# PytorchConnectomics/pytorch_connectomics

Measured on AMD Instinct MI355X. Metric: voxels/s (train + sliding-window infer), MedNeXt-S 112^3 bf16, higher is better.
Workload: dtype bf16; 1 GPU; Lucchi++ sliding-window inference (configs[1]): MedNeXt-S k3, 165x1024x768 volume, roi 112^3, overlap 0.5, bump blending, sw_batch_size 8, random-init weights; step = one whole-volume EagerSlidingWindowEngine call (TTA off); value = window-voxels/s; sw_batch_size=8, window_pipeline_streams=3

## Files before the change

pytorch_connectomics_amd/csrc/dwconv_mfma_kernels.hip:

```cpp
#include <type_traits>

#include "dwconv_march.h"
#include "pw_common.h"

namespace pytc {

typedef short s4_t __attribute__((ext_vector_type(4)));
typedef unsigned int u32x4_t __attribute__((ext_vector_type(4)));
typedef unsigned int u32x2a4_t __attribute__((ext_vector_type(2), aligned(4)));
typedef __bf16 bf2_t __attribute__((ext_vector_type(2)));
typedef float f2_t __attribute__((ext_vector_type(2)));

constexpr int MF_TY = 8, MF_TX = 8, MF_CG = 32;
constexpr int MF_EY = MF_TY + 2, MF_EX = MF_TX + 2;
constexpr int MF_EXP = 16;
constexpr int MF_CS = MF_EY * MF_EXP + 2;
constexpr int MF_IMG = MF_CG * MF_CS;
constexpr int MF_NCHUNK = MF_EY * MF_EX * (MF_CG / 8);
constexpr int MF_CPT = 2;
constexpr int MF_TS = 32;
constexpr int MF_RS = MF_TX * MF_TS + 8;

__device__ __forceinline__ unsigned short mf_bf16_bits(float f) {
  unsigned int u = __float_as_uint(f);
  u += 0x7FFFu + ((u >> 16) & 1u);
  return (unsigned short)(u >> 16);
}
__device__ __forceinline__ float mf_bf16_float(unsigned short h) { return __uint_as_float(((unsigned int)h) << 16); }

template <int N>
__device__ __forceinline__ void mf_wait_vm() { asm volatile("s_waitcnt vmcnt(%0)" : : "n"(N) : "memory"); }


template <int N>
__device__ __forceinline__ void mf_wait_vm_upto(int n) {
  if constexpr (N > 0) {
    if (n >= N) { mf_wait_vm<N>(); return; }
    mf_wait_vm_upto<N - 1>(n);
  } else {
    mf_wait_vm<0>();
  }
}

template <int PF, bool LO, int PROBE = 0, bool STORE = true, int MIXHC = 0>
__global__ void __launch_bounds__(256, MIXHC ? 3 : 4)
dwconv3d_k3_mfma_kernel(const unsigned short* __restrict__ x, unsigned short* __restrict__ y, const float* __restrict__ w,
                        const float* __restrict__ bias, float* __restrict__ stats, DwMarch g, DwMix mx) {
  static_assert(PF == 2 || PF == 3, "two or three planes in flight");
  static_assert(MIXHC == 0 || (STORE && PF == 3), "the fused block keeps the output tile and three planes in flight");
  constexpr bool MIX = MIXHC > 0;
  __shared__ __attribute__((aligned(16))) bf16x8_t w2s[MIX ? MIXHC * 2 * 64 : 1];
  __shared__ __attribute__((aligned(16))) h8_t w3s[MIX ? 2 * MIXHC * 64 : 1];
  __shared__ __attribute__((aligned(16))) float mbias[MIX ? 32 * MIXHC + 32 : 4];
  __shared__ __attribute__((aligned(16))) unsigned short image[2][MF_IMG];
  __shared__ __attribute__((aligned(16))) unsigned short otile[STORE ? 2 : 1][STORE ? MF_TY * MF_RS : 8];
  __shared__ float wl[27 * MF_CG];
  __shared__ float red[4][2][16];

  const int tid = threadIdx.x, wave = tid >> 6, lane = tid & 63;
  int b = g.swizzle ? xcd_swizzle(blockIdx.x, gridDim.x) : blockIdx.x;
  const int ncg = g.C / MF_CG;
  const int cg = g.cg_inner ? b % ncg : (b / g.slots) % ncg;
  const int slot_id = g.cg_inner ? (b / ncg) % g.slots : b % g.slots;
  const int n = b / (ncg * g.slots);
  b = slot_id;
  const int fx = b % g.tx; b /= g.tx;
  const int fy = b % g.ty;
  const int zchunk = b / g.ty;
  const int y0 = fy * MF_TY, x0 = fx * MF_TX;
  const int zs = zchunk * g.zc;
  const int ze = min(zs + g.zc, g.D);
  const int C = g.C;
  const long plane_elems = (long)g.H * g.W * C;
  const unsigned short* xn = x + (long)n * g.D * plane_elems + cg * MF_CG;
  unsigned short* yn = y + (long)n * g.D * plane_elems + cg * MF_CG;
  const bool inner = y0 >= 1 && y0 + MF_TY + 1 <= g.H && x0 >= 1 && x0 + MF_TX + 1 <= g.W;

  for (int i = tid; i < 27 * MF_CG; i += 256) wl[i] = w[(long)(i / MF_CG) * C + cg * MF_CG + (i % MF_CG)];
  if constexpr (MIX) {
    const bf16x8_t* w2g = mx.w2n + (long)n * mx.w2_stride;
    for (int i = tid; i < MIXHC * 2 * 64; i += 256) { w2s[i] = w2g[i]; w3s[i] = mx.w3[i]; }
    if (tid < 32 * MIXHC) mbias[tid] = mx.b2n[(long)n * (32 * MIXHC) + tid];
    else if (tid < 32 * MIXHC + 32) mbias[tid] = mx.b3[tid - 32 * MIXHC];
  }
  __syncthreads();

  int goff[MF_CPT], loff[MF_CPT];
  bool cok[MF_CPT];
#pragma unroll
  for (int i = 0; i < MF_CPT; ++i) {
    const int c = tid + 256 * i;
    const int vox = c >> 2, part = c & 3;
    const int yy = vox / MF_EX, xx = vox % MF_EX;
    const int gy = y0 - 1 + yy, gx = x0 - 1 + xx;
    cok[i] = (c < MF_NCHUNK) && gy >= 0 && gy < g.H && gx >= 0 && gx < g.W;
    const int gyc = min(max(gy, 0), g.H - 1), gxc = min(max(gx, 0), g.W - 1);
    goff[i] = (gyc * g.W + gxc) * C + part * 8;
    loff[i] = (c < MF_NCHUNK) ? (part * 8) * MF_CS + yy * MF_EXP + xx : -1;
  }
  u32x4_t stg[PF][MF_CPT];
  auto issue = [&](int gz, u32x4_t (&st)[MF_CPT]) {
    const int zc = min(max(gz, 0), g.D - 1);
#pragma unroll
    for (int i = 0; i < MF_CPT; ++i) {
      const unsigned short* ptr = xn + (long)zc * plane_elems + goff[i];
      asm volatile("global_load_dwordx4 %0, %1, off" : "=&v"(st[i]) : "v"(ptr) : "memory");
    }
  };
  auto landed = [&](u32x4_t (&st)[MF_CPT], int younger) {
    mf_wait_vm_upto<2 * MF_CPT + 2>(younger);
    asm volatile("" : "+v"(st[0]), "+v"(st[1]) : : "memory");
  };
  auto commit = [&](int slot, u32x4_t (&st)[MF_CPT], int gz) {
    const bool zok = gz >= 0 && gz < g.D;
#pragma unroll
    for (int i = 0; i < MF_CPT; ++i) {
      if (loff[i] < 0) continue;
      unsigned short* dst = &image[slot][loff[i]];
      if (inner && zok) {
#pragma unroll
        for (int q = 0; q < 4; ++q) {
          dst[(2 * q) * MF_CS] = (unsigned short)(st[i][q] & 0xffffu);
          dst[(2 * q + 1) * MF_CS] = (unsigned short)(st[i][q] >> 16);
        }
      } else {
        const bool ok = zok && cok[i];
#pragma unroll
        for (int q = 0; q < 4; ++q) {
          const unsigned int dw = ok ? st[i][q] : 0u;
          dst[(2 * q) * MF_CS] = (unsigned short)(dw & 0xffffu);
          dst[(2 * q + 1) * MF_CS] = (unsigned short)(dw >> 16);
        }
      }
    }
  };

  const int h = wave & 1, ph = wave >> 1;
  const int cl = lane >> 2, j = lane & 3;
  const int ch = h * 16 + cl;
  s4_t a_hi[3][2], a_lo[3][2];
#pragma unroll
  for (int dy = 0; dy < 3; ++dy)
#pragma unroll
    for (int r = 0; r < 2; ++r) {
      s4_t vh, vl;
#pragma unroll
      for (int k = 0; k < 4; ++k) {
        const int i = j;
        const int dz = 2 - i, dx = k - r;
        float wv = 0.f;
        if (i < 3 && dx >= 0 && dx < 3) wv = wl[((dz * 3 + dy) * 3 + dx) * MF_CG + ch];
        const unsigned short hb = mf_bf16_bits(wv);
        vh[k] = (short)hb;
        vl[k] = (short)mf_bf16_bits(wv - mf_bf16_float(hb));
      }
      a_hi[dy][r] = vh;
      a_lo[dy][r] = vl;
    }
  float bv = bias ? bias[cg * MF_CG + ch] : 0.f;
  asm volatile("" : "+v"(bv));

  int boff[4];
  bool pok[4][2];
#pragma unroll
  for (int u = 0; u < 4; ++u) {
    boff[u] = ch * MF_CS + (ph * 4 + j) * MF_EXP + 2 * u;
#pragma unroll
    for (int r = 0; r < 2; ++r) pok[u][r] = (y0 + ph * 4 + j) < g.H && (x0 + 2 * u + r) < g.W;
  }
  const int op = tid >> 2, opiece = tid & 3;
  const int oy = op >> 3, ox = op & 7;
  const bool ook = (y0 + oy) < g.H && (x0 + ox) < g.W;
  const long obase = ((long)(y0 + oy) * g.W + (x0 + ox)) * C + opiece * 8;
  const int orb = oy * MF_RS + ox * MF_TS + opiece * 8;
  int ooff[4];
#pragma unroll
  for (int u = 0; u < 4; ++u) ooff[u] = (ph * 4 + j) * MF_RS + (2 * u) * MF_TS + ch;
  auto flush = [&](int zo) {
    const u32x4_t o = *reinterpret_cast<const u32x4_t*>(&otile[zo & 1][orb]);
    if (ook) *reinterpret_cast<u32x4_t*>(yn + (long)zo * plane_elems + obase) = o;
  };

  const int mr = lane & 15, mkb = lane >> 4;
  const int mp = wave * 16 + mr, my = mp >> 3, mxx = mp & 7;
  const bool mok = (y0 + my) < g.H && (x0 + mxx) < g.W;
  const long mbase = ((long)min(y0 + my, g.H - 1) * g.W + min(x0 + mxx, g.W - 1)) * C + mkb * 8;
  const int mtile = my * MF_RS + mxx * MF_TS + mkb * 8;
  u32x4_t rres[MIX ? 3 : 1];
  auto issue_res = [&](int z, u32x4_t& rr) {
    const unsigned short* ptr = xn + (long)z * plane_elems + mbase;
    asm volatile("global_load_dwordx4 %0, %1, off" : "=&v"(rr) : "v"(ptr) : "memory");
  };
  auto mix = [&](int zo, u32x4_t& rr, int younger) {
    if constexpr (MIX) {
      const bf16x8_t bact = *reinterpret_cast<const bf16x8_t*>(&otile[zo & 1][mtile]);
      f32x4_t acc2[2] = {*reinterpret_cast<const f32x4_t*>(&mbias[32 * MIXHC + mkb * 8]), *reinterpret_cast<const f32x4_t*>(&mbias[32 * MIXHC + mkb * 8 + 4])};
#pragma unroll
      for (int hc = 0; hc < MIXHC; ++hc) {
        f32x4_t acc1[2] = {*reinterpret_cast<const f32x4_t*>(&mbias[hc * 32 + mkb * 8]), *reinterpret_cast<const f32x4_t*>(&mbias[hc * 32 + mkb * 8 + 4])};
#pragma unroll
        for (int mt = 0; mt < 2; ++mt) acc1[mt] = Mma<bf16_t>::mma(w2s[(hc * 2 + mt) * 64 + lane], bact, acc1[mt]);
        float gg[8];
#pragma unroll
        for (int q = 0; q < 4; ++q) { gg[q] = acc1[0][q]; gg[4 + q] = acc1[1][q]; }
        const h8_t bhh = gelu_h8_from_f32(gg);
#pragma unroll
        for (int mo = 0; mo < 2; ++mo) acc2[mo] = __builtin_amdgcn_mfma_f32_16x16x32_f16(w3s[(mo * MIXHC + hc) * 64 + lane], bhh, acc2[mo], 0, 0, 0);
      }
      float v[8];
#pragma unroll
      for (int q = 0; q < 4; ++q) { v[q] = acc2[0][q]; v[4 + q] = acc2[1][q]; }
      if (mx.residual) {
        mf_wait_vm_upto<5>(younger);
        asm volatile("" : "+v"(rr) : : "memory");
        float rv[8];
        VecIO<bf16_t, 8>::load(reinterpret_cast<const bf16_t*>(&rr), rv);
#pragma unroll
        for (int q = 0; q < 8; ++q) v[q] += rv[q];
      }
      const long vo = (long)zo * plane_elems + mbase;
      if (mx.head_w) {
        const bf16x8_t ob = Mma<bf16_t>::from_floats(v);
        if (mx.store_y && mok) *reinterpret_cast<bf16x8_t*>(yn + vo) = ob;
        const f32x4_t hh = Mma<bf16_t>::mma(mx.head_w[lane], ob, f32x4_t{0.f, 0.f, 0.f, 0.f});
        if (mok) {
          float* hy = mx.head_y + ((long)n * g.D * g.H * g.W + (vo - mkb * 8) / C) * mx.n_head;
#pragma unroll
          for (int i = 0; i < 4; ++i)
            if (mkb * 4 + i < mx.n_head) hy[mkb * 4 + i] = hh[i] + (mx.head_b ? mx.head_b[mkb * 4 + i] : 0.f);
        }
      } else if (mok) {
        VecIO<bf16_t, 8>::store(reinterpret_cast<bf16_t*>(yn + vo), v);
      }
    }
  };

  f32x4_t acc[4][2];
#pragma unroll
  for (int u = 0; u < 4; ++u)
#pragma unroll
    for (int r = 0; r < 2; ++r) acc[u][r] = f32x4_t{bv, bv, bv, 0.f};
  float s1 = 0.f, s2 = 0.f;
  unsigned long long tk[9] = {0, 0, 0, 0, 0, 0, 0, 0, 0}, tlast = 0, tstart = 0;
  auto stamp = [&](int k) {
    if constexpr (PROBE == 4) {
      const unsigned long long now = __builtin_amdgcn_s_memtime();
      tk[k] += now - tlast;
      tlast = now;
    }
  };
  if constexpr (PROBE == 4) { tstart = __builtin_amdgcn_s_memtime(); tlast = tstart; }

  auto exists_p = [&](int z) { return z <= ze; };
  auto exists_r = [&](int z) { return MIX && mx.residual && z >= zs && z < ze; };
  auto step = [&](int gz, int slot, u32x4_t (&ld)[MF_CPT], u32x4_t (&cm)[MF_CPT], u32x4_t& rn, u32x4_t& ro) {
    if constexpr (MIX) {
      if (gz - 2 >= zs) mix(gz - 2, ro, (exists_p(gz + 1) ? MF_CPT : 0) + (exists_r(gz - 1) ? 1 : 0) + (exists_p(gz + 2) ? MF_CPT : 0));
      stamp(8);
      if (exists_r(gz)) issue_res(gz, rn);
    } else {
      if (STORE && gz - 2 >= zs && PROBE != 3) flush(gz - 2);
    }
    if (gz + PF <= ze) issue(gz + PF, ld);
    stamp(0);
    const unsigned short* img = image[slot];
#pragma unroll
    for (int dy = 0; dy < ((PROBE == 1 || PROBE == 3) ? 0 : 3); ++dy) {
      s4_t bq[4];
#pragma unroll
      for (int u = 0; u < 4; ++u) bq[u] = __builtin_bit_cast(s4_t, *reinterpret_cast<const u32x2a4_t*>(img + boff[u] + dy * MF_EXP));
#pragma unroll
      for (int u = 0; u < 4; ++u)
#pragma unroll
        for (int r = 0; r < 2; ++r) acc[u][r] = __builtin_amdgcn_mfma_f32_4x4x4bf16_1k(a_hi[dy][r], bq[u], acc[u][r], 0, 0, 0);
      if (LO) {
#pragma unroll
        for (int u = 0; u < 4; ++u)
#pragma unroll
          for (int r = 0; r < 2; ++r) acc[u][r] = __builtin_amdgcn_mfma_f32_4x4x4bf16_1k(a_lo[dy][r], bq[u], acc[u][r], 0, 0, 0);
      }
    }
    stamp(1);
    if (gz + 1 <= ze) {
      landed(cm, MF_CPT * min(PF - 1, ze - gz - 1) + (exists_r(gz - 1) ? 1 : 0) + (exists_r(gz) ? 1 : 0));
      stamp(2);
      commit(slot ^ 1, cm, gz + 1);
      stamp(3);
    } else {
      mf_wait_vm<0>();
    }
    if (gz - 1 >= zs && PROBE != 3) {
      unsigned short* ot = otile[STORE ? (gz - 1) & 1 : 0];
#pragma unroll
      for (int u = 0; u < 4; ++u) {
        const bf2_t hb = __builtin_convertvector(f2_t{acc[u][0][0], acc[u][1][0]}, bf2_t);
        const unsigned int bits = __builtin_bit_cast(unsigned int, hb);
        if constexpr (STORE) {
          ot[ooff[u]] = (unsigned short)(bits & 0xffffu);
          ot[ooff[u] + MF_TS] = (unsigned short)(bits >> 16);
        }
        if constexpr (!MIX) {
          float r0 = __uint_as_float(bits << 16), r1 = __uint_as_float(bits & 0xffff0000u);
          if (!inner) { r0 = pok[u][0] ? r0 : 0.f; r1 = pok[u][1] ? r1 : 0.f; }
          s1 += r0; s2 = fmaf(r0, r0, s2);
          s1 += r1; s2 = fmaf(r1, r1, s2);
        }
      }
    }
#pragma unroll
    for (int u = 0; u < 4; ++u)
#pragma unroll
      for (int r = 0; r < 2; ++r) acc[u][r] = f32x4_t{acc[u][r][1], acc[u][r][2], bv, 0.f};
    stamp(4);
    __syncthreads();
    stamp(5);
    if constexpr (PROBE == 4) tk[6] += 1;
  };

#pragma unroll
  for (int q = 0; q < PF; ++q) issue(zs - 1 + q, stg[q]);
  landed(stg[0], MF_CPT * (PF - 1));
  commit(0, stg[0], zs - 1);
  __syncthreads();
  int slot = 0;
  for (int gz = zs - 1; gz <= ze; gz += PF) {
#pragma unroll
    for (int k = 0; k < PF; ++k) {
      if (gz + k <= ze) { step(gz + k, slot, stg[k], stg[(k + 1) % PF], rres[MIX ? k : 0], rres[MIX ? (k + 1) % 3 : 0]); slot ^= 1; }
    }
  }
  mf_wait_vm<0>();
  if constexpr (MIX) {
    const int rs = (ze - zs) % 3;
    if (rs == 0) mix(ze - 1, rres[0], 0);
    else if (rs == 1) mix(ze - 1, rres[MIX ? 1 : 0], 0);
    else mix(ze - 1, rres[MIX ? 2 : 0], 0);
  } else {
    if (STORE && PROBE != 3) flush(ze - 1);
  }

  if constexpr (PROBE == 4) {
    if constexpr (MIX) {
      if (mx.prof && lane == 0) {
        tk[7] = __builtin_amdgcn_s_memtime() - tstart;
        float* o = mx.prof + (((long)n * g.slots + slot_id) * 4 + wave) * 9;
#pragma unroll
        for (int k = 0; k < 9; ++k) o[k] = (float)tk[k];
      }
    } else if (stats && lane == 0) {
      tk[7] = __builtin_amdgcn_s_memtime() - tstart;
      float* o = stats + (((long)n * g.slots + slot_id) * 2) * C + cg * MF_CG + wave * 8;
#pragma unroll
      for (int k = 0; k < 8; ++k) o[k] = (float)tk[k];
    }
    return;
  }
  if (!MIX && stats) {
    s1 += __shfl_xor(s1, 1, 64); s2 += __shfl_xor(s2, 1, 64);
    s1 += __shfl_xor(s1, 2, 64); s2 += __shfl_xor(s2, 2, 64);
    if (j == 0) { red[wave][0][cl] = s1; red[wave][1][cl] = s2; }
    __syncthreads();
    if (tid < 2 * MF_CG) {
      const int which = tid / MF_CG, chn = tid % MF_CG;
      const float a = red[chn >> 4][which][chn & 15] + red[(chn >> 4) + 2][which][chn & 15];
      stats[(((long)n * g.slots + slot_id) * 2 + which) * C + cg * MF_CG + chn] = a;
    }
  }
}

void dwconv_mfma_launch(const void* x, void* y, const float* w, const float* bias, float* stats, const DwMarch& g, int variant,
                        hipStream_t s) {
  dim3 grid((unsigned)((long)g.slots * (g.C / MF_CG) * g.N)), block(256);
  const unsigned short* xp = (const unsigned short*)x;
  unsigned short* yp = (unsigned short*)y;
  const DwMix none{};
#define PYTC_MF(PFV, LOV, NM) hipLaunchKernelGGL((dwconv3d_k3_mfma_kernel<PFV, LOV, NM>), grid, block, 0, s, xp, yp, w, bias, stats, g, none)
#define PYTC_MF_STATS(PFV, LOV) hipLaunchKernelGGL((dwconv3d_k3_mfma_kernel<PFV, LOV, 0, false>), grid, block, 0, s, xp, yp, w, bias, stats, g, none)
  const int probe = tuning_get("dwconv_mfma_probe", 0);
  if (!y) {
    if (variant & 1) { if (variant & 2) PYTC_MF_STATS(2, true); else PYTC_MF_STATS(3, true); }
    else { if (variant & 2) PYTC_MF_STATS(2, false); else PYTC_MF_STATS(3, false); }
  }
  else if (probe == 1) PYTC_MF(3, false, 1);
  else if (probe == 3) PYTC_MF(3, false, 3);
  else if (probe == 4) PYTC_MF(3, false, 4);
  else if (variant & 1) { if (variant & 2) PYTC_MF(2, true, 0); else PYTC_MF(3, true, 0); }
  else { if (variant & 2) PYTC_MF(2, false, 0); else PYTC_MF(3, false, 0); }
#undef PYTC_MF
#undef PYTC_MF_STATS
}

int dwmix_launch(const void* x, void* y, const float* w, const float* bias, const DwMarch& g, const DwMix& mx, int c_hid, int variant,
                 hipStream_t s) {
  dim3 grid((unsigned)((long)g.slots * g.N)), block(256);
  const unsigned short* xp = (const unsigned short*)x;
  unsigned short* yp = (unsigned short*)y;
#define PYTC_DM(LOV, HCV, PRB) hipLaunchKernelGGL((dwconv3d_k3_mfma_kernel<3, LOV, PRB, true, HCV>), grid, block, 0, s, xp, yp, w, bias, (float*)nullptr, g, mx)
  const bool lo = variant & 1;
  if (mx.prof) {
    if (c_hid != 64 || lo) return -1;
    PYTC_DM(false, 2, 4);
    return 0;
  }
  switch (c_hid) {
    case 64: if (lo) PYTC_DM(true, 2, 0); else PYTC_DM(false, 2, 0); break;
    case 96: if (lo) PYTC_DM(true, 3, 0); else PYTC_DM(false, 3, 0); break;
    case 128: if (lo) PYTC_DM(true, 4, 0); else PYTC_DM(false, 4, 0); break;
    default: return -1;
  }
#undef PYTC_DM
  return 0;
}

}
```

Measured before the change: 1.874 billion voxels/s.

## Add 64-channel workgroup variant of MFMA depthwise conv for large tensors

Templates the depthwise 3D conv MFMA kernel on channel-group width, adding a 64-channel, 512-thread workgroup that handles two 32-channel halves side by side in LDS, padded apart. The launcher picks it by default for tensors with at least 4M elements, or when a tuning knob asks for it. The aim is to halve the grid size and widen the contiguous channel span of each global load and store per voxel. The cost is doubled LDS per block and larger blocks, which may lower occupancy.

```diff
diff --git a/pytorch_connectomics_amd/csrc/dwconv_mfma_kernels.hip b/pytorch_connectomics_amd/csrc/dwconv_mfma_kernels.hip
--- a/pytorch_connectomics_amd/csrc/dwconv_mfma_kernels.hip
+++ b/pytorch_connectomics_amd/csrc/dwconv_mfma_kernels.hip
@@ -16,7 +16,7 @@
 constexpr int MF_EXP = 16;
 constexpr int MF_CS = MF_EY * MF_EXP + 2;
 constexpr int MF_IMG = MF_CG * MF_CS;
-constexpr int MF_NCHUNK = MF_EY * MF_EX * (MF_CG / 8);
+constexpr int MF_HP = 4;
 constexpr int MF_CPT = 2;
 constexpr int MF_TS = 32;
 constexpr int MF_RS = MF_TX * MF_TS + 8;
@@ -42,24 +42,35 @@
   }
 }
 
-template <int PF, bool LO, int PROBE = 0, bool STORE = true, int MIXHC = 0>
-__global__ void __launch_bounds__(256, MIXHC ? 3 : 4)
+template <int PF, bool LO, int PROBE = 0, bool STORE = true, int MIXHC = 0, int CG = MF_CG>
+__global__ void __launch_bounds__(CG * 8, MIXHC ? 3 : 4)
 dwconv3d_k3_mfma_kernel(const unsigned short* __restrict__ x, unsigned short* __restrict__ y, const float* __restrict__ w,
                         const float* __restrict__ bias, float* __restrict__ stats, DwMarch g, DwMix mx) {
   static_assert(PF == 2 || PF == 3, "two or three planes in flight");
   static_assert(MIXHC == 0 || (STORE && PF == 3), "the fused block keeps the output tile and three planes in flight");
+  static_assert(CG == 32 || (CG == 64 && MIXHC == 0), "32 or 64 channels per workgroup; the fused block is C = 32");
   constexpr bool MIX = MIXHC > 0;
+  constexpr int NT = CG * 8;
+  constexpr int NH = CG / MF_CG;
+  constexpr int NPART = CG / 8;
+  constexpr int IMG = MF_IMG + (NH - 1) * (MF_IMG + MF_HP);
+  constexpr int NCHUNK = MF_EY * MF_EX * NPART;
+  constexpr int TS = NH * MF_TS;
+  constexpr int RS = MF_TX * TS + 8;
+  static_assert(CG != MF_CG || RS == MF_RS, "the 32-channel group keeps the layout of tools/lds_conflict_model.py");
+  static_assert(NCHUNK <= MF_CPT * NT, "two chunks per thread cover the haloed plane");
   __shared__ __attribute__((aligned(16))) bf16x8_t w2s[MIX ? MIXHC * 2 * 64 : 1];
   __shared__ __attribute__((aligned(16))) h8_t w3s[MIX ? 2 * MIXHC * 64 : 1];
   __shared__ __attribute__((aligned(16))) float mbias[MIX ? 32 * MIXHC + 32 : 4];
-  __shared__ __attribute__((aligned(16))) unsigned short image[2][MF_IMG];
-  __shared__ __attribute__((aligned(16))) unsigned short otile[STORE ? 2 : 1][STORE ? MF_TY * MF_RS : 8];
-  __shared__ float wl[27 * MF_CG];
-  __shared__ float red[4][2][16];
+  __shared__ __attribute__((aligned(16))) unsigned short image[2][IMG];
+  __shared__ __attribute__((aligned(16))) unsigned short otile[STORE ? 2 : 1][STORE ? MF_TY * RS : 8];
+  __shared__ float wl[27 * CG];
+  __shared__ float red[4 * NH][2][16];
 
   const int tid = threadIdx.x, wave = tid >> 6, lane = tid & 63;
+  const int hh = NH > 1 ? wave >> 2 : 0, hw = NH > 1 ? wave & 3 : wave;
   int b = g.swizzle ? xcd_swizzle(blockIdx.x, gridDim.x) : blockIdx.x;
-  const int ncg = g.C / MF_CG;
+  const int ncg = g.C / CG;
   const int cg = g.cg_inner ? b % ncg : (b / g.slots) % ncg;
   const int slot_id = g.cg_inner ? (b / ncg) % g.slots : b % g.slots;
   const int n = b / (ncg * g.slots);
@@ -72,11 +83,11 @@
   const int ze = min(zs + g.zc, g.D);
   const int C = g.C;
   const long plane_elems = (long)g.H * g.W * C;
-  const unsigned short* xn = x + (long)n * g.D * plane_elems + cg * MF_CG;
-  unsigned short* yn = y + (long)n * g.D * plane_elems + cg * MF_CG;
+  const unsigned short* xn = x + (long)n * g.D * plane_elems + cg * CG;
+  unsigned short* yn = y + (long)n * g.D * plane_elems + cg * CG;
   const bool inner = y0 >= 1 && y0 + MF_TY + 1 <= g.H && x0 >= 1 && x0 + MF_TX + 1 <= g.W;
 
-  for (int i = tid; i < 27 * MF_CG; i += 256) wl[i] = w[(long)(i / MF_CG) * C + cg * MF_CG + (i % MF_CG)];
+  for (int i = tid; i < 27 * CG; i += NT) wl[i] = w[(long)(i / CG) * C + cg * CG + (i % CG)];
   if constexpr (MIX) {
     const bf16x8_t* w2g = mx.w2n + (long)n * mx.w2_stride;
     for (int i = tid; i < MIXHC * 2 * 64; i += 256) { w2s[i] = w2g[i]; w3s[i] = mx.w3[i]; }
@@ -89,14 +100,14 @@
   bool cok[MF_CPT];
 #pragma unroll
   for (int i = 0; i < MF_CPT; ++i) {
-    const int c = tid + 256 * i;
-    const int vox = c >> 2, part = c & 3;
+    const int c = tid + NT * i;
+    const int vox = c / NPART, part = c % NPART;
     const int yy = vox / MF_EX, xx = vox % MF_EX;
     const int gy = y0 - 1 + yy, gx = x0 - 1 + xx;
-    cok[i] = (c < MF_NCHUNK) && gy >= 0 && gy < g.H && gx >= 0 && gx < g.W;
+    cok[i] = (c < NCHUNK) && gy >= 0 && gy < g.H && gx >= 0 && gx < g.W;
     const int gyc = min(max(gy, 0), g.H - 1), gxc = min(max(gx, 0), g.W - 1);
     goff[i] = (gyc * g.W + gxc) * C + part * 8;
-    loff[i] = (c < MF_NCHUNK) ? (part * 8) * MF_CS + yy * MF_EXP + xx : -1;
+    loff[i] = (c < NCHUNK) ? (part >> 2) * (MF_IMG + MF_HP) + ((part & 3) * 8) * MF_CS + yy * MF_EXP + xx : -1;
   }
   u32x4_t stg[PF][MF_CPT];
   auto issue = [&](int gz, u32x4_t (&st)[MF_CPT]) {
@@ -135,9 +146,10 @@
     }
   };
 
-  const int h = wave & 1, ph = wave >> 1;
+  const int h = hw & 1, ph = hw >> 1;
   const int cl = lane >> 2, j = lane & 3;
   const int ch = h * 16 + cl;
+  const int chg = hh * MF_CG + ch;
   s4_t a_hi[3][2], a_lo[3][2];
 #pragma unroll
   for (int dy = 0; dy < 3; ++dy)
@@ -149,7 +161,7 @@
         const int i = j;
         const int dz = 2 - i, dx = k - r;
         float wv = 0.f;
-        if (i < 3 && dx >= 0 && dx < 3) wv = wl[((dz * 3 + dy) * 3 + dx) * MF_CG + ch];
+        if (i < 3 && dx >= 0 && dx < 3) wv = wl[((dz * 3 + dy) * 3 + dx) * CG + chg];
         const unsigned short hb = mf_bf16_bits(wv);
         vh[k] = (short)hb;
         vl[k] = (short)mf_bf16_bits(wv - mf_bf16_float(hb));
@@ -157,35 +169,35 @@
       a_hi[dy][r] = vh;
       a_lo[dy][r] = vl;
     }
-  float bv = bias ? bias[cg * MF_CG + ch] : 0.f;
+  float bv = bias ? bias[cg * CG + chg] : 0.f;
   asm volatile("" : "+v"(bv));
 
   int boff[4];
   bool pok[4][2];
 #pragma unroll
   for (int u = 0; u < 4; ++u) {
-    boff[u] = ch * MF_CS + (ph * 4 + j) * MF_EXP + 2 * u;
+    boff[u] = hh * (MF_IMG + MF_HP) + ch * MF_CS + (ph * 4 + j) * MF_EXP + 2 * u;
 #pragma unroll
     for (int r = 0; r < 2; ++r) pok[u][r] = (y0 + ph * 4 + j) < g.H && (x0 + 2 * u + r) < g.W;
   }
-  const int op = tid >> 2, opiece = tid & 3;
+  const int op = tid / NPART, opiece = tid % NPART;
   const int oy = op >> 3, ox = op & 7;
   const bool ook = (y0 + oy) < g.H && (x0 + ox) < g.W;
   const long obase = ((long)(y0 + oy) * g.W + (x0 + ox)) * C + opiece * 8;
-  const int orb = oy * MF_RS + ox * MF_TS + opiece * 8;
+  const int orb = oy * RS + ox * TS + opiece * 8;
   int ooff[4];
 #pragma unroll
-  for (int u = 0; u < 4; ++u) ooff[u] = (ph * 4 + j) * MF_RS + (2 * u) * MF_TS + ch;
+  for (int u = 0; u < 4; ++u) ooff[u] = (ph * 4 + j) * RS + (2 * u) * TS + chg;
   auto flush = [&](int zo) {
     const u32x4_t o = *reinterpret_cast<const u32x4_t*>(&otile[zo & 1][orb]);
     if (ook) *reinterpret_cast<u32x4_t*>(yn + (long)zo * plane_elems + obase) = o;
   };
 
   const int mr = lane & 15, mkb = lane >> 4;
-  const int mp = wave * 16 + mr, my = mp >> 3, mxx = mp & 7;
+  const int mp = hw * 16 + mr, my = mp >> 3, mxx = mp & 7;
   const bool mok = (y0 + my) < g.H && (x0 + mxx) < g.W;
   const long mbase = ((long)min(y0 + my, g.H - 1) * g.W + min(x0 + mxx, g.W - 1)) * C + mkb * 8;
-  const int mtile = my * MF_RS + mxx * MF_TS + mkb * 8;
+  const int mtile = my * RS + mxx * TS + mkb * 8;
   u32x4_t rres[MIX ? 3 : 1];
   auto issue_res = [&](int z, u32x4_t& rr) {
     const unsigned short* ptr = xn + (long)z * plane_elems + mbase;
@@ -297,7 +309,7 @@
         const unsigned int bits = __builtin_bit_cast(unsigned int, hb);
         if constexpr (STORE) {
           ot[ooff[u]] = (unsigned short)(bits & 0xffffu);
-          ot[ooff[u] + MF_TS] = (unsigned short)(bits >> 16);
+          ot[ooff[u] + TS] = (unsigned short)(bits >> 16);
         }
         if constexpr (!MIX) {
           float r0 = __uint_as_float(bits << 16), r1 = __uint_as_float(bits & 0xffff0000u);
@@ -349,7 +361,7 @@
       }
     } else if (stats && lane == 0) {
       tk[7] = __builtin_amdgcn_s_memtime() - tstart;
-      float* o = stats + (((long)n * g.slots + slot_id) * 2) * C + cg * MF_CG + wave * 8;
+      float* o = stats + (((long)n * g.slots + slot_id) * 2) * C + cg * CG + wave * 8;
 #pragma unroll
       for (int k = 0; k < 8; ++k) o[k] = (float)tk[k];
     }
@@ -360,23 +372,28 @@
     s1 += __shfl_xor(s1, 2, 64); s2 += __shfl_xor(s2, 2, 64);
     if (j == 0) { red[wave][0][cl] = s1; red[wave][1][cl] = s2; }
     __syncthreads();
-    if (tid < 2 * MF_CG) {
-      const int which = tid / MF_CG, chn = tid % MF_CG;
-      const float a = red[chn >> 4][which][chn & 15] + red[(chn >> 4) + 2][which][chn & 15];
-      stats[(((long)n * g.slots + slot_id) * 2 + which) * C + cg * MF_CG + chn] = a;
+    if (tid < 2 * CG) {
+      const int which = tid / CG, chn = tid % CG;
+      const int rw = (chn >> 5) * 4 + ((chn >> 4) & 1);
+      const float a = red[rw][which][chn & 15] + red[rw + 2][which][chn & 15];
+      stats[(((long)n * g.slots + slot_id) * 2 + which) * C + cg * CG + chn] = a;
     }
   }
 }
 
 void dwconv_mfma_launch(const void* x, void* y, const float* w, const float* bias, float* stats, const DwMarch& g, int variant,
                         hipStream_t s) {
-  dim3 grid((unsigned)((long)g.slots * (g.C / MF_CG) * g.N)), block(256);
+  const int probe = y ? tuning_get("dwconv_mfma_probe", 0) : 0;
+  const int cgk = tuning_get("dwconv_mfma_cg", 0);
+  const bool cg64 = g.C % 64 == 0 && probe == 0 && (cgk == 64 || (cgk != 32 && (long)g.D * g.H * g.W * g.C >= (4L << 20)));
+  const int cgn = cg64 ? 64 : MF_CG;
+  dim3 grid((unsigned)((long)g.slots * (g.C / cgn) * g.N)), block(cgn * 8);
   const unsigned short* xp = (const unsigned short*)x;
   unsigned short* yp = (unsigned short*)y;
   const DwMix none{};
-#define PYTC_MF(PFV, LOV, NM) hipLaunchKernelGGL((dwconv3d_k3_mfma_kernel<PFV, LOV, NM>), grid, block, 0, s, xp, yp, w, bias, stats, g, none)
-#define PYTC_MF_STATS(PFV, LOV) hipLaunchKernelGGL((dwconv3d_k3_mfma_kernel<PFV, LOV, 0, false>), grid, block, 0, s, xp, yp, w, bias, stats, g, none)
-  const int probe = tuning_get("dwconv_mfma_probe", 0);
+#define PYTC_MF_CG(PFV, LOV, NM, ST, CGV) hipLaunchKernelGGL((dwconv3d_k3_mfma_kernel<PFV, LOV, NM, ST, 0, CGV>), grid, block, 0, s, xp, yp, w, bias, stats, g, none)
+#define PYTC_MF(PFV, LOV, NM) do { if (cg64) PYTC_MF_CG(PFV, LOV, 0, true, 64); else PYTC_MF_CG(PFV, LOV, NM, true, 32); } while (0)
+#define PYTC_MF_STATS(PFV, LOV) do { if (cg64) PYTC_MF_CG(PFV, LOV, 0, false, 64); else PYTC_MF_CG(PFV, LOV, 0, false, 32); } while (0)
   if (!y) {
     if (variant & 1) { if (variant & 2) PYTC_MF_STATS(2, true); else PYTC_MF_STATS(3, true); }
     else { if (variant & 2) PYTC_MF_STATS(2, false); else PYTC_MF_STATS(3, false); }
@@ -388,6 +405,7 @@
   else { if (variant & 2) PYTC_MF(2, false, 0); else PYTC_MF(3, false, 0); }
 #undef PYTC_MF
 #undef PYTC_MF_STATS
+#undef PYTC_MF_CG
 }
 
 int dwmix_launch(const void* x, void* y, const float* w, const float* bias, const DwMarch& g, const DwMix& mx, int c_hid, int variant,
```

Result: no change. 1.886 billion voxels/s (median of 6 runs) (+0.6%).
